# OlegArenz/gmmvi

Measured on AMD Instinct MI355X. Metric: samples_components_per_sec, higher is better.
Workload: dtype f32; 1 GPU; ns: stm target D=20, K=100 components (100/GPU), 100 samples/component, N=10000 samples/iter, SAMTRON (Stein, fixed K, reuse ratio 0, KL trust regions, improvement-based stepsizes); K=100, D=20, N=10000, parallelism=component-shard x1

## Files before the change

gmmvi_amd/csrc/stein.hip:

```cpp
#include "common.h"
#include "blocked.h"
#include "wave_reduce.h"
#include "stein_finalize.h"
#include "stein_tile.h"
#include <cstdlib>

typedef float f32x4 __attribute__((ext_vector_type(4)));

__device__ __forceinline__ float wave_max(float v) { return gmmvi_wave_max(v); }

template <int DP>
__global__ __launch_bounds__(1024) void stein_finalize_kernel(int D, int R, int N, int flags, const float* __restrict__ part,
                                                             const float* __restrict__ part_m, float* __restrict__ H_neg,
                                                             float* __restrict__ g_neg, const float* __restrict__ packed) {
    extern __shared__ float fin_lds[];
    stein_finalize_component<DP>(fin_lds, blockIdx.x, D, R, N, flags, part, part_m, H_neg, g_neg, packed);
}

template <int DP>
static int launch_stein_finalize(gmmvi_ctx* ctx, int K, int D, int R, int N, int flags, const float* part,
                                 const float* part_m, float* H_neg, float* g_neg, const float* packed) {
    const size_t shmem = stein_finalize_lds_floats(DP, D, R) * sizeof(float);
    int rc = gmmvi_ensure_dynamic_lds(ctx, (const void*)stein_finalize_kernel<DP>, shmem);
    if (rc != GMMVI_OK) return rc;
    const int threads = Pack<DP>::FRAGS ? 1024 : 256;
    GMMVI_PROF(ctx, "stein_finalize");
    hipLaunchKernelGGL(stein_finalize_kernel<DP>, dim3(K), dim3(threads), shmem, ctx->stream, D, R, N, flags, part, part_m, H_neg,
                       g_neg, packed);
    GMMVI_LAUNCH_CHECK(ctx);
    return GMMVI_OK;
}

template <int DP, int VW>
__device__ __forceinline__ void sm_load_row(const float* __restrict__ row, int D, float (&v)[DP]) {
#pragma unroll
    for (int f = 0; f < DP; f += VW) {
        if (VW > 1 || f < SteinTile<DP>::PREV + 1 || f < D) {
            if constexpr (VW == 4) {
                const float4 t = *reinterpret_cast<const float4*>(row + f);
                v[f] = t.x; v[f + 1] = t.y; v[f + 2] = t.z; v[f + 3] = t.w;
            } else if constexpr (VW == 2) {
                const float2 t = *reinterpret_cast<const float2*>(row + f);
                v[f] = t.x; v[f + 1] = t.y;
            } else {
                v[f] = row[f];
            }
        } else {
            v[f] = 0.f;
        }
    }
}

template <int DP, bool EXACT>
__device__ __forceinline__ void sm_store_rows(float* t, int D, const float (&v)[DP]) {
#pragma unroll
    for (int f = 0; f < DP; ++f)
        if (EXACT || f < SteinTile<DP>::PREV + 1 || f < D) t[f * SM_RS] = v[f];
}

template <int DP, int VW>
__global__ __launch_bounds__(256, (SteinTile<DP>::MT <= 2 ? 2 : 1))
void stein_moment_kernel(int K, int D_rt, int N, int wave_range, int stacks, int R, const float* __restrict__ packed,
                         const float* __restrict__ X, const float* __restrict__ TG, const float* __restrict__ QG,
                         const float* __restrict__ ld, const float* __restrict__ bg, const int32_t* __restrict__ mapping,
                         int map_offset, int own_rt, float* __restrict__ part, float* __restrict__ part_m) {
    using ST = SteinTile<DP>;
    constexpr int MT = ST::MT, NT = ST::NT, NB = ST::NB;
    constexpr bool EXACT = VW > 1;
    const int D = EXACT ? DP : D_rt;
    const bool own = EXACT ? false : own_rt != 0;
    extern __shared__ float sm[];
    __shared__ float sm_m[4][NB];
    const int tid = threadIdx.x;
    const int lane = tid & 63;
    const int wave = __builtin_amdgcn_readfirstlane(tid >> 6);
    const int D1 = D + 1;
    const int per_xcd = (stacks * R + 7) / 8;
    const int item = ((int)blockIdx.x & 7) * per_xcd + ((int)blockIdx.x >> 3);
    if (item >= stacks * R) return;
    const int range_id = item / stacks;
    const int k0 = (item - range_id * stacks) * NB;
    const int nb = min(NB, K - k0);
    const int rows_g = D1 + 1, rows_x = D1;
    constexpr int rows_e = NB + 1;
    const int wave_floats = (rows_g + rows_x + rows_e) * SM_RS;
    const int wave_stride = max(wave_floats, 16 * MT * (16 * NT + 1));
    float* Tg = sm + (size_t)wave * wave_stride;
    float* Tx = Tg + rows_g * SM_RS;
    float* Te = Tx + rows_x * SM_RS;
    for (int e = lane; e < SM_RS; e += 64) { Tg[D1 * SM_RS + e] = 0.f; Te[NB * SM_RS + e] = 0.f; Tx[D * SM_RS + e] = 1.f; }

    const int q = lane >> 4, c16 = lane & 15;
    int a_off[MT], x_off[NT], e_off[NT], cidx[NT];
    float mu[NT];
#pragma unroll
    for (int mt = 0; mt < MT; ++mt) {
        const int row = 16 * mt + c16;
        a_off[mt] = (row < D1 ? row : D1) * SM_RS + 4 * q;
    }
#pragma unroll
    for (int nt = 0; nt < NT; ++nt) {
        const int c = 16 * nt + c16;
        const int comp = c / D1, j = c - comp * D1;
        const bool valid = comp < nb;
        cidx[nt] = valid ? comp : NB;
        x_off[nt] = (valid ? j : 0) * SM_RS + 4 * q;
        e_off[nt] = (valid ? comp : NB) * SM_RS + 4 * q;
        mu[nt] = (valid && j < D) ? packed[(size_t)(k0 + comp) * Pack<DP>::STRIDE + j] : 0.f;
    }
    const int w_begin = min(N, (range_id * 4 + wave) * wave_range);
    const int w_end = min(N, w_begin + wave_range);

    float c_lim[NB];
#pragma unroll
    for (int c = 0; c < NB; ++c) c_lim[c] = c < nb ? 3.0e38f : -3.0e38f;
    auto log_weights = [&](int n0, float (&a)[NB]) {
        const int n = min(n0 + lane, N - 1);
        const float lim = (n0 + lane < w_end) ? 3.0e38f : -3.0e38f;
        if (own) {
            const int mp = mapping[n] + map_offset;
#pragma unroll
            for (int c = 0; c < NB; ++c) a[c] = fminf((mp == k0 + c) ? 0.f : -3.0e38f, fminf(lim, c_lim[c]));
        } else {
            const float bgv = bg[n];
#pragma unroll
            for (int c = 0; c < NB; ++c) a[c] = fminf(ld[(size_t)min(k0 + c, K - 1) * N + n] - bgv, fminf(lim, c_lim[c]));
        }
    };

    float a[NB], xr[DP], tr[DP], qr[DP];
    auto fetch = [&](int n0) {
        const size_t row = (size_t)min(n0 + lane, N - 1) * D;
        log_weights(n0, a);
        sm_load_row<DP, VW>(X + row, D, xr);
        sm_load_row<DP, VW>(TG + row, D, tr);
        sm_load_row<DP, VW>(QG + row, D, qr);
    };
    if (MT >= 4 && w_begin < w_end) fetch(w_begin);

    float M[NB];
#pragma unroll
    for (int c = 0; c < NB; ++c) M[c] = -3.0e38f;
    for (int n0 = w_begin; n0 < w_end; n0 += 64) {
        float a1[NB];
        log_weights(n0, a1);
#pragma unroll
        for (int c = 0; c < NB; ++c) M[c] = fmaxf(M[c], a1[c]);
    }
#pragma unroll
    for (int c = 0; c < NB; ++c) M[c] = wave_max(M[c]);

    f32x4 acc[MT][NT];
#pragma unroll
    for (int mt = 0; mt < MT; ++mt)
#pragma unroll
        for (int nt = 0; nt < NT; ++nt)
#pragma unroll
            for (int r = 0; r < 4; ++r) acc[mt][nt][r] = 0.f;
    if (MT < 4 && w_begin < w_end) fetch(w_begin);
    for (int n0 = w_begin; n0 < w_end; n0 += 64) {
        const int n_here = min(64, w_end - n0);
        sm_store_rows<DP, EXACT>(Tx + lane, D, xr);
#pragma unroll
        for (int f = 0; f < DP; ++f) tr[f] -= qr[f];
        sm_store_rows<DP, EXACT>(Tg + lane, D, tr);
#pragma unroll
        for (int c = 0; c < NB; ++c) Te[c * SM_RS + lane] = (a[c] > -1.0e38f) ? __expf(a[c] - M[c]) : 0.f;
        Tg[D * SM_RS + lane] = 1.f;
        WAVE_LDS_SYNC();
        fetch(n0 + 64);
#pragma unroll
        for (int u = 0; u < 4; ++u) {
            if (16 * u < n_here) {
                f32x4 av[MT], bv[NT];
#pragma unroll
                for (int mt = 0; mt < MT; ++mt) av[mt] = *reinterpret_cast<const f32x4*>(Tg + a_off[mt] + 16 * u);
#pragma unroll
                for (int nt = 0; nt < NT; ++nt) {
                    const f32x4 xv = *reinterpret_cast<const f32x4*>(Tx + x_off[nt] + 16 * u);
                    const f32x4 ev = *reinterpret_cast<const f32x4*>(Te + e_off[nt] + 16 * u);
                    bv[nt] = (xv - mu[nt]) * ev;
                }
#pragma unroll
                for (int sp = 0; sp < 4; ++sp)
#pragma unroll
                    for (int mt = 0; mt < MT; ++mt)
#pragma unroll
                        for (int nt = 0; nt < NT; ++nt)
                            acc[mt][nt] = __builtin_amdgcn_mfma_f32_16x16x4f32(av[mt][sp], bv[nt][sp], acc[mt][nt], 0, 0, 0);
            }
        }
        WAVE_LDS_SYNC();
    }

    if constexpr (MT >= 4) {
        constexpr int CW = 16 * NT + 1;
        float* C = sm + (size_t)wave * wave_stride;
    #pragma unroll
        for (int nt = 0; nt < NT; ++nt)
    #pragma unroll
            for (int mt = 0; mt < MT; ++mt)
    #pragma unroll
                for (int r = 0; r < 4; ++r) C[(16 * mt + 4 * q + r) * CW + 16 * nt + c16] = acc[mt][nt][r];
        if (lane == 0) {
    #pragma unroll
            for (int c = 0; c < NB; ++c) sm_m[wave][c] = M[c];
        }
        __syncthreads();
        const int DD = D1 * D1;
    #pragma unroll
        for (int c = 0; c < NB; ++c) {
            if (c < nb) {
                const float m0 = sm_m[0][c], m1 = sm_m[1][c], m2 = sm_m[2][c], m3 = sm_m[3][c];
                const float Mall = fmaxf(fmaxf(m0, m1), fmaxf(m2, m3));
                const float f0 = __expf(m0 - Mall), f1 = __expf(m1 - Mall), f2 = __expf(m2 - Mall), f3 = __expf(m3 - Mall);
                float* dst = part + ((size_t)(k0 + c) * R + range_id) * DD;
                for (int el = tid; el < DD; el += 256) {
                    const int i = el / D1, j = el - i * D1;
                    const float* src = sm + i * CW + c * D1 + j;
                    dst[el] = fmaf(src[3 * wave_stride], f3, fmaf(src[2 * wave_stride], f2, fmaf(src[wave_stride], f1, src[0] * f0)));
                }
                if (tid == 0) part_m[(size_t)(k0 + c) * R + range_id] = Mall;
            }
        }
    } else {
        if (lane == 0) {
    #pragma unroll
            for (int c = 0; c < NB; ++c) sm_m[wave][c] = M[c];
        }
        __syncthreads();
        float Mall[NB], fsc[NB];
    #pragma unroll
        for (int c = 0; c < NB; ++c) {
            Mall[c] = fmaxf(fmaxf(sm_m[0][c], sm_m[1][c]), fmaxf(sm_m[2][c], sm_m[3][c]));
            fsc[c] = __expf(M[c] - Mall[c]);
        }
        constexpr int CW = 16 * NT + 1;
        float* C = sm;
        for (int w = 0; w < 4; ++w) {
            if (wave == w) {
    #pragma unroll
                for (int nt = 0; nt < NT; ++nt) {
                    float fs = 1.f;
    #pragma unroll
                    for (int c = 0; c < NB; ++c) fs = (cidx[nt] == c) ? fsc[c] : fs;
    #pragma unroll
                    for (int mt = 0; mt < MT; ++mt)
    #pragma unroll
                        for (int r = 0; r < 4; ++r) {
                            float* dst = C + (16 * mt + 4 * q + r) * CW + 16 * nt + c16;
                            const float v = acc[mt][nt][r] * fs;
                            *dst = (w == 0) ? v : *dst + v;
                        }
                }
            }
            __syncthreads();
        }
        const int DD = D1 * D1;
        for (int el = tid; el < nb * DD; el += 256) {
            const int comp = el / DD, rem = el - comp * DD;
            const int i = rem / D1, j = rem - i * D1;
            part[((size_t)(k0 + comp) * R + range_id) * DD + rem] = C[i * CW + comp * D1 + j];
        }
        if (tid < nb) part_m[(size_t)(k0 + tid) * R + range_id] = Mall[tid];
    }
}

template <int DP, int VW>
static int launch_stein_moment(gmmvi_ctx* ctx, int K, int D, const float* packed, const float* X, int N, const float* ld,
                               const float* qgrad, const float* bg, const float* tgrad, const int32_t* mapping,
                               int map_offset, int flags, float* H_neg, float* g_neg, SteinSlab* slab_out) {
    using ST = SteinTile<DP>;
    const int D1 = D + 1;
    const int stacks = (K + ST::NB - 1) / ST::NB;
    const int wgs_per_cu = ST::MT == 1 ? 2 : 1;
    static const int env_wgs = getenv("GMMVI_STEIN_WGS_PER_CU") ? atoi(getenv("GMMVI_STEIN_WGS_PER_CU")) : 0;
    int R = ((env_wgs > 0 ? env_wgs : wgs_per_cu) * ctx->num_cus) / stacks;
    if (R > (N + 255) / 256) R = (N + 255) / 256;
    if (R < 1) R = 1;
    int wave_range = (((N + R - 1) / R + 3) / 4 + 3) / 4 * 4;
    R = (N + 4 * wave_range - 1) / (4 * wave_range);
    const size_t part_floats = (size_t)K * R * D1 * D1;
    int rc = gmmvi_ws_reserve(ctx, (part_floats + (size_t)K * R) * sizeof(float));
    if (rc != GMMVI_OK) return rc;
    float* part = (float*)ctx->ws;
    float* part_m = part + part_floats;
    const int per_xcd = (stacks * R + 7) / 8;
    {
        size_t floats = (size_t)(2 * D1 + ST::NB + 2) * SM_RS;
        if (floats < (size_t)16 * ST::MT * (16 * ST::NT + 1)) floats = (size_t)16 * ST::MT * (16 * ST::NT + 1);
        const size_t shmem = 4 * floats * sizeof(float);
        rc = gmmvi_ensure_dynamic_lds(ctx, (const void*)stein_moment_kernel<DP, VW>, shmem);
        if (rc != GMMVI_OK) return rc;
        GMMVI_PROF(ctx, "stein_partial");
        hipLaunchKernelGGL((stein_moment_kernel<DP, VW>), dim3(8 * per_xcd), dim3(256), shmem, ctx->stream, K, D, N, wave_range,
                           stacks, R, packed, X, tgrad, qgrad, ld, bg, mapping, map_offset,
                           (flags & GMMVI_OWN_SAMPLES_ONLY) ? 1 : 0, part, part_m);
    }
    GMMVI_LAUNCH_CHECK(ctx);
    if (slab_out != nullptr) {
        slab_out->part = part; slab_out->part_m = part_m; slab_out->R = R;
        return GMMVI_OK;
    }
    return launch_stein_finalize<DP>(ctx, K, D, R, N, flags, part, part_m, H_neg, g_neg, packed);
}

static int stein_moment(gmmvi_ctx* ctx, int K, int D, const float* packed, const float* X, int N, const float* ld,
                        const float* qgrad, const float* bg, const float* tgrad, const int32_t* mapping, int map_offset,
                        int flags, float* H_neg, float* g_neg, SteinSlab* slab_out) {
    const int dp = gmmvi_padded_dim(D);
    const uintptr_t bases = reinterpret_cast<uintptr_t>(X) | reinterpret_cast<uintptr_t>(tgrad) | reinterpret_cast<uintptr_t>(qgrad);
    const int vw_nat = (dp % 4 == 0) ? 4 : 2;
    const bool fast = D == dp && !(flags & GMMVI_OWN_SAMPLES_ONLY) && bases % (4 * vw_nat) == 0;
#define GMMVI_SM(DPV)                                                                                                  \
    case DPV:                                                                                                          \
        if (fast)                                                                                                      \
            return launch_stein_moment<DPV, (DPV % 4 == 0 ? 4 : 2)>(ctx, K, D, packed, X, N, ld, qgrad, bg, tgrad, mapping, \
                                                                    map_offset, flags, H_neg, g_neg, slab_out);         \
        return launch_stein_moment<DPV, 1>(ctx, K, D, packed, X, N, ld, qgrad, bg, tgrad, mapping, map_offset, flags, H_neg, g_neg, slab_out)
    switch (dp) {
        GMMVI_SM(2); GMMVI_SM(4); GMMVI_SM(8); GMMVI_SM(10); GMMVI_SM(12); GMMVI_SM(16); GMMVI_SM(20); GMMVI_SM(24);
        GMMVI_SM(32); GMMVI_SM(40); GMMVI_SM(50); GMMVI_SM(64);
        default: break;
    }
#undef GMMVI_SM
    return gmmvi_fail(ctx, GMMVI_ERR_ARG, "gmmvi_stein: unsupported dimension (D must be <= 63)");
}

extern "C" int gmmvi_stein(gmmvi_ctx* ctx, int K, int D, const float* packed_dev, const float* X_dev, int N,
                           const float* ld_dev, const float* qgrad_dev, const float* bg_dev, const float* tgrad_dev,
                           const int32_t* mapping_dev, int map_offset, int flags, float* H_neg_out_dev,
                           float* g_neg_out_dev) {
    GMMVI_ARG_CHECK(ctx, K >= 1 && D >= 1 && (D < GMMVI_MAX_DIM || gmmvi_is_blocked_dim(D)) && N >= 1);
    GMMVI_ARG_CHECK(ctx, packed_dev && X_dev && qgrad_dev && tgrad_dev && H_neg_out_dev && g_neg_out_dev);
    if (flags & GMMVI_OWN_SAMPLES_ONLY) GMMVI_ARG_CHECK(ctx, mapping_dev != nullptr);
    else GMMVI_ARG_CHECK(ctx, ld_dev && bg_dev);
    if (gmmvi_is_blocked_dim(D))
        return gmmvi_blocked_stein(ctx, K, D, packed_dev, X_dev, N, ld_dev, qgrad_dev, bg_dev, tgrad_dev, mapping_dev,
                                   map_offset, flags, H_neg_out_dev, g_neg_out_dev);
    return stein_moment(ctx, K, D, packed_dev, X_dev, N, ld_dev, qgrad_dev, bg_dev, tgrad_dev, mapping_dev, map_offset, flags,
                        H_neg_out_dev, g_neg_out_dev, nullptr);
}

int gmmvi_stein_partials(gmmvi_ctx* ctx, int K, int D, const float* packed_dev, const float* X_dev, int N, const float* ld_dev,
                         const float* qgrad_dev, const float* bg_dev, const float* tgrad_dev, int flags, SteinSlab* slab) {
    GMMVI_ARG_CHECK(ctx, K >= 1 && D >= 1 && D < GMMVI_MAX_DIM && !gmmvi_is_blocked_dim(D) && N >= 1 && slab != nullptr);
    GMMVI_ARG_CHECK(ctx, packed_dev && X_dev && qgrad_dev && tgrad_dev && ld_dev && bg_dev && !(flags & GMMVI_OWN_SAMPLES_ONLY));
    return stein_moment(ctx, K, D, packed_dev, X_dev, N, ld_dev, qgrad_dev, bg_dev, tgrad_dev, nullptr, 0, flags, nullptr, nullptr,
                        slab);
}

int gmmvi_stein_finalize_slab(gmmvi_ctx* ctx, int K, int D, const SteinSlab& slab, int N, int flags, const float* packed_dev,
                              float* H_neg_out_dev, float* g_neg_out_dev) {
    switch (gmmvi_padded_dim(D)) {
#define GMMVI_FIN(DPV) case DPV: return launch_stein_finalize<DPV>(ctx, K, D, slab.R, N, flags, slab.part, slab.part_m,       \
                                                                  H_neg_out_dev, g_neg_out_dev, packed_dev)
        GMMVI_FIN(2); GMMVI_FIN(4); GMMVI_FIN(8); GMMVI_FIN(10); GMMVI_FIN(12); GMMVI_FIN(16); GMMVI_FIN(20); GMMVI_FIN(24);
        GMMVI_FIN(32); GMMVI_FIN(40); GMMVI_FIN(50); GMMVI_FIN(64);
#undef GMMVI_FIN
        default: return gmmvi_fail(ctx, GMMVI_ERR_ARG, "stein_finalize: unsupported dimension");
    }
}
```

gmmvi_amd/csrc/stein_tile.h:

```cpp
#pragma once
#include "common.h"

#define WAVE_LDS_SYNC()                                        \
    do {                                                       \
        asm volatile("s_waitcnt lgkmcnt(0)" ::: "memory");     \
        __builtin_amdgcn_wave_barrier();                       \
    } while (0)


constexpr int SM_RS = 72;
constexpr int SM_NBMAX = 5;

template <int DP>
struct SteinTile {
    static constexpr int D1 = DP + 1 < 64 ? DP + 1 : 64;
    static constexpr int MT = (D1 + 15) / 16;
    static constexpr int NTMAX = MT <= 2 ? 6 : (MT == 3 ? 6 : 7);
    static constexpr int pick_nt() {
        int best = 1;
        long best_num = 0, best_den = 1;
        for (int nt = 1; nt <= NTMAX; ++nt) {
            int nb = (16 * nt) / D1;
            if (nb > SM_NBMAX) nb = SM_NBMAX;
            if (nb < 1) continue;
            const long num = (long)nb * D1, den = 16L * nt;
            if (num * best_den > best_num * den) { best = nt; best_num = num; best_den = den; }
        }
        return best;
    }
    static constexpr int NT = pick_nt();
    static constexpr int NB = (16 * NT) / D1 < SM_NBMAX ? (16 * NT) / D1 : SM_NBMAX;
    static constexpr int PREV = DP == 2 ? 0 : DP == 4 ? 2 : DP == 8 ? 4 : DP == 10 ? 8 : DP == 12 ? 10 : DP == 16 ? 12 : DP == 20 ? 16
                                : DP == 24 ? 20 : DP == 32 ? 24 : DP == 40 ? 32 : DP == 50 ? 40 : 50;
};
```

Measured before the change: 4.856 billion samples*components/s.

## Replace sparse last MFMA row tile with VALU FMAs and 4x4 MFMA tail

When the last 16-row M tile of the Stein moment GEMM holds only a few valid rows (D1=21 leaves 5 rows), that tile is no longer computed with full 16x16x4 MFMAs. The first four tail rows use 4x4x1 MFMAs and the remaining row uses per-lane VALU FMAs or adds. The partial sums are then reduced with cross-lane shuffles and written back into the accumulator layout. The aim is to avoid spending MFMA work on padding rows. The cost is extra VALU work, shuffles and more register pressure.

New measurement: 4.280 billion samples*components/s. 0.881x the previous value.

```diff
diff --git a/gmmvi_amd/csrc/stein.hip b/gmmvi_amd/csrc/stein.hip
--- a/gmmvi_amd/csrc/stein.hip
+++ b/gmmvi_amd/csrc/stein.hip
@@ -58,6 +58,15 @@
         if (EXACT || f < SteinTile<DP>::PREV + 1 || f < D) t[f * SM_RS] = v[f];
 }
 
+__device__ __forceinline__ float sm_fma(float a, float b, float c) {
+    asm("v_fma_f32 %0, %1, %2, %0" : "+v"(c) : "v"(a), "v"(b));
+    return c;
+}
+__device__ __forceinline__ float sm_add(float c, float b) {
+    asm("v_add_f32 %0, %1, %0" : "+v"(c) : "v"(b));
+    return c;
+}
+
 template <int DP, int VW>
 __global__ __launch_bounds__(256, (SteinTile<DP>::MT <= 2 ? 2 : 1))
 void stein_moment_kernel(int K, int D_rt, int N, int wave_range, int stacks, int R, const float* __restrict__ packed,
@@ -66,6 +75,7 @@
                          int map_offset, int own_rt, float* __restrict__ part, float* __restrict__ part_m) {
     using ST = SteinTile<DP>;
     constexpr int MT = ST::MT, NT = ST::NT, NB = ST::NB;
+    constexpr int MTM = ST::MT_MFMA, TAIL = ST::TAIL, T4 = ST::TAIL4, TL = TAIL ? TAIL : 1;
     constexpr bool EXACT = VW > 1;
     const int D = EXACT ? DP : D_rt;
     const bool own = EXACT ? false : own_rt != 0;
@@ -91,13 +101,20 @@
     for (int e = lane; e < SM_RS; e += 64) { Tg[D1 * SM_RS + e] = 0.f; Te[NB * SM_RS + e] = 0.f; Tx[D * SM_RS + e] = 1.f; }
 
     const int q = lane >> 4, c16 = lane & 15;
-    int a_off[MT], x_off[NT], e_off[NT], cidx[NT];
+    int a_off[MTM], t_off[TL], x_off[NT], e_off[NT], cidx[NT];
     float mu[NT];
 #pragma unroll
-    for (int mt = 0; mt < MT; ++mt) {
+    for (int mt = 0; mt < MTM; ++mt) {
         const int row = 16 * mt + c16;
         a_off[mt] = (row < D1 ? row : D1) * SM_RS + 4 * q;
     }
+#pragma unroll
+    for (int r = 0; r < TL; ++r) {
+        const int row = 16 * (MT - 1) + r;
+        t_off[r] = (row < D1 ? row : D1) * SM_RS + 4 * q;
+    }
+    const int row4 = 16 * (MT - 1) + (c16 & 3);
+    const int t4_off = (row4 < D1 ? row4 : D1) * SM_RS + 4 * q;
 #pragma unroll
     for (int nt = 0; nt < NT; ++nt) {
         const int c = 16 * nt + c16;
@@ -157,6 +174,16 @@
         for (int nt = 0; nt < NT; ++nt)
 #pragma unroll
             for (int r = 0; r < 4; ++r) acc[mt][nt][r] = 0.f;
+    float tl[TL][NT];
+#pragma unroll
+    for (int r = 0; r < TL; ++r)
+#pragma unroll
+        for (int nt = 0; nt < NT; ++nt) tl[r][nt] = 0.f;
+    f32x4 t4[T4 ? NT : 1];
+#pragma unroll
+    for (int nt = 0; nt < (T4 ? NT : 1); ++nt)
+#pragma unroll
+        for (int r = 0; r < 4; ++r) t4[nt][r] = 0.f;
     if (MT < 4 && w_begin < w_end) fetch(w_begin);
     for (int n0 = w_begin; n0 < w_end; n0 += 64) {
         const int n_here = min(64, w_end - n0);
@@ -172,9 +199,14 @@
 #pragma unroll
         for (int u = 0; u < 4; ++u) {
             if (16 * u < n_here) {
-                f32x4 av[MT], bv[NT];
-#pragma unroll
-                for (int mt = 0; mt < MT; ++mt) av[mt] = *reinterpret_cast<const f32x4*>(Tg + a_off[mt] + 16 * u);
+                f32x4 av[MTM], bv[NT], gv[TL];
+#pragma unroll
+                for (int mt = 0; mt < MTM; ++mt) av[mt] = *reinterpret_cast<const f32x4*>(Tg + a_off[mt] + 16 * u);
+#pragma unroll
+                for (int r = T4; r < TAIL; ++r)
+                    if (!EXACT || r < TAIL - 1) gv[r] = *reinterpret_cast<const f32x4*>(Tg + t_off[r] + 16 * u);
+                f32x4 g4;
+                if constexpr (T4 > 0) g4 = *reinterpret_cast<const f32x4*>(Tg + t4_off + 16 * u);
 #pragma unroll
                 for (int nt = 0; nt < NT; ++nt) {
                     const f32x4 xv = *reinterpret_cast<const f32x4*>(Tx + x_off[nt] + 16 * u);
@@ -182,15 +214,47 @@
                     bv[nt] = (xv - mu[nt]) * ev;
                 }
 #pragma unroll
-                for (int sp = 0; sp < 4; ++sp)
-#pragma unroll
-                    for (int mt = 0; mt < MT; ++mt)
+                for (int sp = 0; sp < 4; ++sp) {
+#pragma unroll
+                    for (int mt = 0; mt < MTM; ++mt)
 #pragma unroll
                         for (int nt = 0; nt < NT; ++nt)
                             acc[mt][nt] = __builtin_amdgcn_mfma_f32_16x16x4f32(av[mt][sp], bv[nt][sp], acc[mt][nt], 0, 0, 0);
+                    if constexpr (T4 > 0) {
+#pragma unroll
+                        for (int nt = 0; nt < NT; ++nt)
+                            t4[nt] = __builtin_amdgcn_mfma_f32_4x4x1f32(g4[sp], bv[nt][sp], t4[nt], 0, 0, 0);
+                    }
+#pragma unroll
+                    for (int r = T4; r < TAIL; ++r)
+#pragma unroll
+                        for (int nt = 0; nt < NT; ++nt)
+                            tl[r][nt] = (EXACT && r == TAIL - 1) ? sm_add(tl[r][nt], bv[nt][sp])
+                                                                 : sm_fma(gv[r][sp], bv[nt][sp], tl[r][nt]);
+                }
             }
         }
         WAVE_LDS_SYNC();
+    }
+
+    if constexpr (TAIL > 0) {
+#pragma unroll
+        for (int nt = 0; nt < NT; ++nt) {
+            float s[TL];
+#pragma unroll
+            for (int r = 0; r < TAIL; ++r) {
+                s[r] = r < T4 ? t4[T4 ? nt : 0][r & 3] : tl[r][nt];
+                s[r] = s[r] + __shfl_xor(s[r], 16);
+                s[r] = s[r] + __shfl_xor(s[r], 32);
+            }
+#pragma unroll
+            for (int r = 0; r < 4; ++r) {
+                float v = 0.f;
+                if (r < TAIL) v = (q == 0) ? s[r] : v;
+                if (r + 4 < TAIL) v = (q == 1) ? s[r + 4] : v;
+                acc[MT - 1][nt][r] = v;
+            }
+        }
     }
 
     if constexpr (MT >= 4) {
diff --git a/gmmvi_amd/csrc/stein_tile.h b/gmmvi_amd/csrc/stein_tile.h
--- a/gmmvi_amd/csrc/stein_tile.h
+++ b/gmmvi_amd/csrc/stein_tile.h
@@ -30,6 +30,11 @@
     }
     static constexpr int NT = pick_nt();
     static constexpr int NB = (16 * NT) / D1 < SM_NBMAX ? (16 * NT) / D1 : SM_NBMAX;
+    static constexpr int TAIL_MAX = 5;
+    static constexpr int LAST_ROWS = D1 - 16 * (MT - 1);
+    static constexpr int TAIL = (MT >= 2 && LAST_ROWS <= TAIL_MAX) ? LAST_ROWS : 0;
+    static constexpr int MT_MFMA = TAIL ? MT - 1 : MT;
+    static constexpr int TAIL4 = TAIL == 5 ? 4 : 0;
     static constexpr int PREV = DP == 2 ? 0 : DP == 4 ? 2 : DP == 8 ? 4 : DP == 10 ? 8 : DP == 12 ? 10 : DP == 16 ? 12 : DP == 20 ? 16
                                 : DP == 24 ? 20 : DP == 32 ? 24 : DP == 40 ? 32 : DP == 50 ? 40 : 50;
 };
```
